# kevlar-dev/kevlar

Measured on AMD Instinct MI355X. Metric: reads/sec through count+novel (3 samples, k=31), higher is better.
Workload: dtype u64 hash / u8 counters

## Files before the change

### kevlar_amd/csrc/kv_binned.hip

```cpp
#include <algorithm>
#include <cmath>
#include <map>
#include <type_traits>

#include "kv_binned.h"
#include "kv_device.h"
#include "kv_kmer2bit_device.h"

namespace {

#define BIN_RING_MIN 64
#define BIN_RING_MAX 4096
#define BIN_B_THREADS 512
#define BIN_B_ITEMS 8
#define BIN_B_BUDGET 16384
#define BIN_C_THREADS 1024
#define BIN_MAX_SEG 512

template <typename ItemT>
struct Rings {
    ItemT *ring;
    uint32_t *cnt, *base;
    uint32_t R;
    uint32_t skew;
// ... 263 lines not shown
        __syncthreads();
        const uint64_t i0 = next_chunk * chunk;
        if (i0 >= n) break;
        uint64_t idx = i0 + threadIdx.x;
        uint64_t h_next = idx < n ? list[idx * stride] : 0, c_next = (W && idx < n) ? list[idx * stride + 1] : 1;
        for (int round = 0; round < BIN_LIST_ROUNDS; ++round) {
            const uint64_t h = h_next, count = c_next;
            const bool live = idx < n;
            idx += THREADS;
            if (round + 1 < BIN_LIST_ROUNDS && idx < n) {
                h_next = list[idx * stride];
                if (W) c_next = list[idx * stride + 1];
            }
            if (!live) continue;
            n_added += count;
            uint32_t left = W ? (uint32_t)min(count, (uint64_t)255) : 1u;
            while (left) {
                const uint32_t wgt = W ? min(left, BIN_W_MAX) : 1u;
                left -= wgt;
                uint32_t sidx[BIN_MAX_T], item[BIN_MAX_T], pos[BIN_MAX_T];
                uint64_t bins[BIN_MAX_T];
#pragma unroll
                for (int t = 0; t < BIN_MAX_T; ++t) {
                    if (t >= g.T) break;
                    const uint64_t bin = fastmod(h, sk->size[t], sk->magic[t]);
                    const uint32_t slice = (uint32_t)(bin >> g.sbits);
                    const uint32_t c = g.F == 1 ? slice : __umulhi(slice, g.recipF);
                    bins[t] = bin;
                    item[t] = ((slice - c * (uint32_t)g.F) << g.sbits) | ((uint32_t)bin & ((1u << g.sbits) - 1u)) | (W ? (wgt - 1u) << BIN_W_SHIFT : 0u);
                    sidx[t] = (uint32_t)t * (uint32_t)g.C + c;
                }
#pragma unroll
                for (int t = 0; t < BIN_MAX_T; ++t)
                    if (t < g.T) pos[t] = atomicAdd(&cur[sidx[t]], 1u);
#pragma unroll
                for (int t = 0; t < BIN_MAX_T; ++t) {
                    if (t >= g.T) break;
                    if (pos[t] < g.cap1) g.gbuf1[((uint64_t)sidx[t] * g.nwgA + blockIdx.x) * g.cap1 + pos[t]] = item[t];
                    else spill_item(g, t, bins[t], wgt);
                }
            }
        }
    }
    __syncthreads();
    for (uint32_t s = threadIdx.x; s < ns; s += THREADS)
        g.gcnt1[(uint64_t)s * g.nwgA + blockIdx.x] = (uint32_t)min((uint64_t)cur[s], g.cap1);
    if (W) {
        n_added = wave_sum_u64(n_added);
        if ((threadIdx.x & 63) == 0 && n_added) atomicAdd(&g.ctr[2], (unsigned long long)n_added);
    }
}

template <bool W>
__global__ __launch_bounds__(BIN_B_THREADS) void k_bin_split(BinGeom g)
{
    typedef typename std::conditional<W, uint32_t, uint16_t>::type Out;
    extern __shared__ __attribute__((aligned(16))) unsigned char smem[];
    const uint32_t s = blockIdx.y;
    const uint32_t t = s / (uint32_t)g.C, c = s % (uint32_t)g.C;
    const uint32_t F = (uint32_t)g.F;
    Rings<Out> rs;
    rs.R = g.ringB;
    rs.skew = 8;
    rs.ring = (Out *)smem;
    rs.cnt = (uint32_t *)(smem + (((size_t)F * rs.R * sizeof(Out) + 15) & ~(size_t)15));
    rs.base = rs.cnt + F;
    for (uint32_t i = threadIdx.x; i < F; i += BIN_B_THREADS) { rs.cnt[i] = 0; rs.base[i] = 0; }
    __syncthreads();
    uint32_t written = 0;
    uint64_t seg_base = 0;
    {
        const uint32_t nwaves = BIN_B_THREADS >> 6, per_wave = (F + nwaves - 1) / nwaves;
        const uint32_t mine = (threadIdx.x >> 6) * per_wave + (threadIdx.x & 63);
        if ((threadIdx.x & 63) < per_wave && mine < F) seg_base = (((uint64_t)s * F + mine) * g.nwgB + blockIdx.x) * g.cap2;
    }
    Out *gbuf2 = (Out *)g.gbuf2;
    constexpr uint32_t SB = BIN_SLICE_BITS, OFFMASK = (1u << SB) - 1u;
    auto slice_of = [](uint32_t item) { return W ? (item >> SB) & ((1u << (BIN_W_SHIFT - SB)) - 1u) : item >> SB; };
    auto fine_of = [](uint32_t item) { return W ? (Out)((item & OFFMASK) | (((item >> BIN_W_SHIFT) + 1u) << 16)) : (Out)(item & OFFMASK); };
    auto spill_coarse = [&](uint32_t item) {
        spill_item(g, (int)t, (((uint64_t)c * F + slice_of(item)) << SB) | (item & OFFMASK), W ? (item >> BIN_W_SHIFT) + 1u : 1u);
    };
    auto store = [&](uint64_t idx, Out off) { gbuf2[idx] = off; };
    auto overflow = [&](uint32_t fi, Out off) {
        spill_item(g, (int)t, (((uint64_t)c * F + fi) << SB) | ((uint32_t)off & OFFMASK), W ? (uint32_t)off >> 16 : 1u);
    };
    constexpr int ITEMS = W ? 4 : BIN_B_ITEMS;
    const uint64_t step = (uint64_t)BIN_B_THREADS * ITEMS;
    for (uint32_t seg = blockIdx.x; seg < g.nwgA; seg += g.nwgB) {
        uint64_t end = g.gcnt1[(uint64_t)s * g.nwgA + seg];
        if (end > g.cap1) end = g.cap1;
        const uint32_t *src = g.gbuf1 + ((uint64_t)s * g.nwgA + seg) * g.cap1;
        uint4 va = make_uint4(0, 0, 0, 0), vb = va;
        auto fetch = [&](uint64_t r0, uint4 &a, uint4 &b) {
            const uint64_t i0 = r0 + (uint64_t)threadIdx.x * ITEMS;
            if (i0 + ITEMS <= end) { a = *(const uint4 *)(src + i0); if (ITEMS == 8) b = *(const uint4 *)(src + i0 + 4); }
        };
        fetch(0, va, vb);
        for (uint64_t r0 = 0; r0 < end; r0 += step) {
            const uint64_t i0 = r0 + (uint64_t)threadIdx.x * ITEMS;
            uint32_t items[ITEMS];
            int have = 0;
            if (i0 + ITEMS <= end) {
                items[0] = va.x; items[1] = va.y; items[2] = va.z; items[3] = va.w;
                if (ITEMS == 8) { items[ITEMS - 4] = vb.x; items[ITEMS - 3] = vb.y; items[ITEMS - 2] = vb.z; items[ITEMS - 1] = vb.w; }
                have = ITEMS;
            } else {
                for (uint64_t i = i0; i < end; ++i) items[have++] = src[i];
            }
            if (r0 + step < end) fetch(r0 + step, va, vb);
            if (have == ITEMS) {
                uint32_t pos[ITEMS], rbase[ITEMS];
#pragma unroll
                for (int j = 0; j < ITEMS; ++j) pos[j] = atomicAdd(&rs.cnt[slice_of(items[j])], 1u);
#pragma unroll
                for (int j = 0; j < ITEMS; ++j) rbase[j] = rs.base[slice_of(items[j])];
                uint32_t full = 0;
#pragma unroll
                for (int j = 0; j < ITEMS; ++j) {
                    const uint32_t fi = slice_of(items[j]);
                    if (pos[j] - rbase[j] < rs.R) rs.ring[fi * rs.R + ((pos[j] + rs.skew * fi) & (rs.R - 1))] = fine_of(items[j]);
                    else full |= 1u << j;
                }
                if (full) {
#pragma unroll
                    for (int j = 0; j < ITEMS; ++j)
                        if (full & (1u << j)) spill_coarse(items[j]);
                }
            } else {
                for (int j = 0; j < have; ++j)
                    if (!ring_append(rs, slice_of(items[j]), fine_of(items[j]))) spill_coarse(items[j]);
            }
            __syncthreads();
            rings_flush_lanes(rs, F, written, seg_base, (uint32_t)g.cap2, gbuf2, overflow);
            __syncthreads();
        }
    }
    rings_flush(rs, F, true, written, seg_base, (uint32_t)g.cap2, store, overflow, 64u / (uint32_t)sizeof(Out));
    rings_store_counts(F, written, (uint32_t)g.cap2, g.gcnt2 + (uint64_t)s * F * g.nwgB, g.nwgB, blockIdx.x);
}

__device__ __forceinline__ bool lds_inc(uint32_t *lds, uint32_t off, int storage)
{
    if (storage == ST_BIT) {
        const uint32_t bit = 1u << (off & 31);
        return (atomicOr(&lds[off >> 5], bit) & bit) == 0;
    }
    uint32_t *w;
    uint32_t shift, maxv;
    if (storage == ST_BYTE) {
        w = &lds[off >> 2]; shift = (off & 3) * 8u; maxv = 255u;
    } else {
        const uint32_t byte = off >> 1;
        w = &lds[byte >> 2]; shift = (byte & 3) * 8u + ((off & 1) ? 0u : 4u); maxv = 15u;
    }
    uint32_t old = *w;
    for (;;) {
        const uint32_t cur = (old >> shift) & maxv;
        if (cur == maxv) return false;
        const uint32_t prev = atomicCAS(w, old, old + (1u << shift));
        if (prev == old) return cur == 0;
        old = prev;
    }
}

template <int STORAGE>
__device__ __forceinline__ uint32_t lds_inc8(uint32_t *lds, const uint32_t (&w)[4], uint32_t n)
{
    uint32_t fresh = 0;
    if (STORAGE == ST_BIT) {
#pragma unroll
        for (int e = 0; e < 8; ++e) {
            const uint32_t off = (e & 1) ? (w[e >> 1] >> 16) : (w[e >> 1] & 0xffffu);
            if ((uint32_t)e < n) {
                const uint32_t bit = 1u << (off & 31);
                fresh += (atomicOr(&lds[off >> 5], bit) & bit) == 0 ? 1u : 0u;
            }
        }
        return fresh;
    }
    constexpr uint32_t maxv = STORAGE == ST_BYTE ? 255u : 15u;
    uint32_t widx[8], inc[8], old[8], prev[8];
    uint32_t retry = 0;
#pragma unroll
    for (int e = 0; e < 8; ++e) {
        const uint32_t off = (e & 1) ? (w[e >> 1] >> 16) : (w[e >> 1] & 0xffffu);
        uint32_t shift;
        if (STORAGE == ST_BYTE) { widx[e] = off >> 2; shift = (off & 3u) << 3; }
        else { widx[e] = off >> 3; shift = (((off >> 1) & 3u) << 3) + ((off & 1u) ? 0u : 4u); }
        inc[e] = 1u << shift;
    }
#pragma unroll
// ... 39 lines not shown
        for (int e = 0; e < 4; ++e) {
            const uint32_t off = w[e] & 0xffffu;
            if ((uint32_t)e < n) {
                const uint32_t bit = 1u << (off & 31);
                fresh += (atomicOr(&lds[off >> 5], bit) & bit) == 0 ? 1u : 0u;
            }
        }
        return fresh;
    }
    constexpr uint32_t maxv = STORAGE == ST_BYTE ? 255u : 15u;
    uint32_t widx[4], shift[4], add[4], old[4], prev[4];
    bool live[4];
    uint32_t retry = 0;
#pragma unroll
    for (int e = 0; e < 4; ++e) {
        const uint32_t off = w[e] & 0xffffu;
        add[e] = w[e] >> 16;
        if (STORAGE == ST_BYTE) { widx[e] = off >> 2; shift[e] = (off & 3u) << 3; }
        else { widx[e] = off >> 3; shift[e] = (((off >> 1) & 3u) << 3) + ((off & 1u) ? 0u : 4u); }
    }
#pragma unroll
    for (int e = 0; e < 4; ++e) old[e] = lds[widx[e]];
#pragma unroll
    for (int e = 0; e < 4; ++e) {
        const uint32_t field = (old[e] >> shift[e]) & maxv;
        const uint32_t nf = min(maxv, field + add[e]);
        live[e] = (uint32_t)e < n && nf != field;
        prev[e] = atomicCAS(&lds[widx[e]], old[e], old[e] + (live[e] ? (nf - field) << shift[e] : 0u));
    }
#pragma unroll
    for (int e = 0; e < 4; ++e) {
        const bool won = prev[e] == old[e];
        fresh += (live[e] && won && ((old[e] >> shift[e]) & maxv) == 0) ? 1u : 0u;
        retry |= (live[e] && !won) ? (1u << e) : 0u;
    }
    if (retry) {
#pragma unroll
        for (int e = 0; e < 4; ++e) {
            if (!(retry & (1u << e))) continue;
            uint32_t cur_word = prev[e];
            for (;;) {
                const uint32_t field = (cur_word >> shift[e]) & maxv;
                if (field == maxv) break;
                const uint32_t nf = min(maxv, field + add[e]);
                const uint32_t seen = atomicCAS(&lds[widx[e]], cur_word, cur_word + ((nf - field) << shift[e]));
                if (seen == cur_word) { fresh += field == 0 ? 1u : 0u; break; }
                cur_word = seen;
            }
        }
    }
    return fresh;
}

template <int STORAGE, bool W>
__global__ __launch_bounds__(BIN_C_THREADS) void k_bin_apply(const SketchDev *__restrict__ sk, BinGeom g)
{
    typedef typename std::conditional<W, uint32_t, uint16_t>::type Item;
    constexpr uint32_t VEC = 16u / sizeof(Item);
    constexpr uint32_t SB = BIN_SLICE_BITS, SLICE = 1u << SB;
    constexpr uint32_t THREADS = BIN_C_THREADS;
    constexpr int MAXV = W ? 4 : 3;
    __shared__ __attribute__((aligned(16))) uint32_t lds[SLICE / 4];
    const int t = blockIdx.y;
    const uint32_t slice = blockIdx.x;
    if (slice >= g.nslices[t]) return;
    const uint32_t c = slice / (uint32_t)g.F, fidx = slice % (uint32_t)g.F;
    const uint64_t stream = ((uint64_t)t * g.C + c) * g.F + fidx;
    constexpr int storage = STORAGE;
    const uint64_t bin0 = (uint64_t)slice << SB;
    const uint64_t left = g.tsize[t] - bin0, nb = left < SLICE ? left : SLICE;
    const uint64_t byte0 = storage == ST_BYTE ? bin0 : (storage == ST_NIBBLE ? bin0 >> 1 : bin0 >> 3);
    const uint64_t nbytes = storage == ST_BYTE ? nb : (storage == ST_NIBBLE ? (nb + 1) / 2 : (nb + 7) / 8);
    const uint32_t nvec = (uint32_t)((nbytes + 15) / 16);
    uint4 *tab = (uint4 *)(g.ttab[t] + byte0);
    uint4 *l4 = (uint4 *)lds;
    __shared__ uint32_t seg_cnt[BIN_MAX_SEG], vpre[BIN_MAX_SEG];
    __shared__ uint16_t segof[MAXV * THREADS];
    __shared__ uint32_t wsum[THREADS / 64];
    __shared__ uint32_t total_vec_sh, flag_sh, fresh_sh;
    const Item *items = (const Item *)g.gbuf2 + stream * g.nwgB * g.cap2;
    const uint32_t *counts = g.gcnt2 + stream * g.nwgB;
    {
        uint32_t myc = 0;
        if (threadIdx.x < g.nwgB) myc = counts[threadIdx.x];
        unsigned long long flag = 0;
        if (threadIdx.x == THREADS - 1) flag = g.ctr[1];
        if (!g.zero_tables)
            for (uint32_t j = threadIdx.x; j < nvec; j += THREADS) l4[j] = tab[j];
        if (threadIdx.x < g.nwgB) seg_cnt[threadIdx.x] = myc;
        const uint32_t myv = (myc + VEC - 1) / VEC;
        const int lane = threadIdx.x & 63, wave = threadIdx.x >> 6;
        uint32_t incl = myv;
#pragma unroll
        for (int d = 1; d < 64; d <<= 1) {
            const uint32_t up = __shfl_up(incl, d);
            if (lane >= d) incl += up;
        }
        if (lane == 63) wsum[wave] = incl;
        if (threadIdx.x == THREADS - 1) { flag_sh = flag != 0 ? 1u : 0u; fresh_sh = 0; }
        __syncthreads();
        uint32_t before = 0;
        for (int w = 0; w < wave; ++w) before += wsum[w];
        if (threadIdx.x < g.nwgB) vpre[threadIdx.x] = before + incl - myv;
        if (threadIdx.x == THREADS - 1) total_vec_sh = before + incl;
        __syncthreads();
        for (uint32_t sgi = (uint32_t)wave; sgi < g.nwgB; sgi += THREADS / 64) {
            const uint32_t first = vpre[sgi], nv = (seg_cnt[sgi] + VEC - 1) / VEC;
            for (uint32_t i = (uint32_t)lane; i < nv && first + i < (uint32_t)MAXV * THREADS; i += 64) segof[first + i] = (uint16_t)sgi;
        }
        __syncthreads();
    }
    if (flag_sh) return;
    const uint32_t total_vec = total_vec_sh;
    if (total_vec == 0) {
        if (g.zero_tables)
            for (uint32_t j = threadIdx.x; j < nvec; j += THREADS) tab[j] = make_uint4(0, 0, 0, 0);
        return;
    }
    struct Vec { uint4 q; uint32_t n; };
    auto fetch = [&](uint32_t v) {
        Vec r;
        r.q = make_uint4(0, 0, 0, 0); r.n = 0;
        if (v >= total_vec) return r;
        uint32_t lo = 0, hi = g.nwgB;
        if (v < (uint32_t)MAXV * THREADS) {
            lo = segof[v];
        } else {
            while (hi - lo > 1) {
                const uint32_t mid = (lo + hi) >> 1;
                if (vpre[mid] <= v) lo = mid; else hi = mid;
            }
        }
        const uint32_t j0 = (v - vpre[lo]) * VEC;
        r.n = min(VEC, seg_cnt[lo] - j0);
        r.q = *(const uint4 *)(items + (uint64_t)lo * g.cap2 + j0);
        return r;
    };
    Vec first[MAXV];
#pragma unroll
    for (int i = 0; i < MAXV; ++i) first[i] = fetch(threadIdx.x + (uint32_t)i * THREADS);
    if (g.zero_tables)
        for (uint32_t j = threadIdx.x; j < nvec; j += THREADS) l4[j] = make_uint4(0, 0, 0, 0);
    __syncthreads();
    uint32_t fresh = 0;
#pragma unroll
    for (int i = 0; i < MAXV; ++i) {
        const uint32_t w[4] = {first[i].q.x, first[i].q.y, first[i].q.z, first[i].q.w};
        if (first[i].n) fresh += W ? lds_addw4<STORAGE>(lds, w, first[i].n) : lds_inc8<STORAGE>(lds, w, first[i].n);
    }
    if (total_vec > (uint32_t)MAXV * THREADS) {
        const uint32_t v_start = (uint32_t)MAXV * THREADS + threadIdx.x;
        Vec v0 = fetch(v_start), v1 = fetch(v_start + THREADS);
        for (uint32_t v = v_start; v < total_vec; v += THREADS) {
            const Vec v2 = fetch(v + 2 * THREADS);
            const uint32_t w[4] = {v0.q.x, v0.q.y, v0.q.z, v0.q.w};
            fresh += W ? lds_addw4<STORAGE>(lds, w, v0.n) : lds_inc8<STORAGE>(lds, w, v0.n);
            v0 = v1; v1 = v2;
        }
    }
    if (t == 0) {
        const uint32_t tot = (uint32_t)wave_sum_u64(fresh);
        if ((threadIdx.x & 63) == 0 && tot) atomicAdd(&fresh_sh, tot);
    }
    __syncthreads();
    for (uint32_t j = threadIdx.x; j < nvec; j += THREADS) tab[j] = l4[j];
    if (t == 0 && threadIdx.x == 0 && fresh_sh) atomicAdd(&g.ctr[3], (unsigned long long)fresh_sh);
}

__device__ __forceinline__ bool table_add_bin(const SketchDev *s, int t, uint64_t bin, uint32_t weight)
{
    uint8_t *tab = s->tab[t];
    if (s->storage == ST_BIT) {
        const uint32_t bit = 1u << (bin & 31);
        return (atomicOr((uint32_t *)tab + (bin >> 5), bit) & bit) == 0;
    }
    uint32_t *w;
    uint32_t shift, maxv;
    if (s->storage == ST_BYTE) {
        w = (uint32_t *)(tab + (bin & ~3ull)); shift = (uint32_t)(bin & 3) * 8u; maxv = 255u;
    } else {
        const uint64_t byte = bin >> 1;
        w = (uint32_t *)(tab + (byte & ~3ull)); shift = (uint32_t)(byte & 3) * 8u + ((bin & 1) ? 0u : 4u); maxv = 15u;
    }
    uint32_t old = __hip_atomic_load(w, __ATOMIC_RELAXED, __HIP_MEMORY_SCOPE_AGENT);
    for (;;) {
        const uint32_t cur = (old >> shift) & maxv;
        if (cur == maxv) return false;
        const uint32_t nf = min(maxv, cur + weight);
        const uint32_t prev = atomicCAS(w, old, old + ((nf - cur) << shift));
        if (prev == old) return cur == 0;
        old = prev;
    }
}

__global__ void k_bin_spill(const SketchDev *__restrict__ sk, BinGeom g)
{
    if (g.ctr[1] != 0) return;
    unsigned long long n = g.ctr[0];
    if (n > g.spill_cap) n = g.spill_cap;
    uint64_t fresh = 0;
    for (uint64_t i = blockIdx.x * (uint64_t)blockDim.x + threadIdx.x; i < n; i += (uint64_t)gridDim.x * blockDim.x) {
        const unsigned long long e = g.spill[i];
        const int t = (int)((e >> 32) & 0xffu);
        const bool was_zero = table_add_bin(sk, t, e & 0xffffffffull, (uint32_t)((e >> 40) & 0xffu) + 1u);
        fresh += (was_zero && t == 0) ? 1 : 0;
    }
    fresh = wave_sum_u64(fresh);
    if ((threadIdx.x & 63) == 0 && fresh) atomicAdd(&g.ctr[3], (unsigned long long)fresh);
}

std::map<hipStream_t, KvArena> g_scratch;
std::mutex g_scratch_mu;

KvArena &scratch_for(hipStream_t st)
{
    std::lock_guard<std::mutex> lk(g_scratch_mu);
    return g_scratch[kv_stream_key(st)];
}
}
void kv_bin_scratch_release()
{
    std::lock_guard<std::mutex> lk(g_scratch_mu);
    for (auto &kv : g_scratch) kv.second.release();
}
namespace {

template <typename K>
void ensure_dynamic_lds(K kernel, size_t bytes) { kv_ensure_dynamic_lds((const void *)kernel, bytes); }

}

int kv_device_cus()
{
    static int cus = 0;
    if (cus == 0) {
        int dev = 0, n = 256;
        kv_thread_device();
        (void)hipGetDevice(&dev);
        (void)hipDeviceGetAttribute(&n, hipDeviceAttributeMultiprocessorCount, dev);
        cus = n;
    }
    return cus;
}

double kv_estimate_distinct(uint64_t occupied, uint64_t size)
{
    if (occupied >= size) return (double)size * std::log((double)size);
    return -(double)size * std::log1p(-(double)occupied / (double)size);
}

bool kv_bin_two_bit(const kv_sketch *s, const kv_reads *reads)
{
    const char *e = kv_knob("KV_BIN_2BIT");
    if (e && atoi(e) == 0) return false;
    return reads && reads->uni_len != 0 && reads->uni_per_tile != 0 && s->h.hashfam == HF_MURMUR && s->h.ksize >= SKM_MIN_K && s->h.ksize <= SKM_MAX_K &&
           reads->uni_len >= (uint32_t)s->h.ksize && reads->n_tiles > 0;
}

bool kv_binned_eligible(const kv_sketch *s, const kv_reads *reads, uint64_t n_kmers, int nbands)
{
    const char *force = kv_knob("KV_COUNT_PATH");
    if (force && strcmp(force, "atomic") == 0) return false;
    if (s->h.ntables > BIN_MAX_T) return false;
    uint64_t pmin = UINT64_MAX, pmax = 0;
    for (int t = 0; t < s->h.ntables; ++t) { pmin = std::min(pmin, s->h.size[t]); pmax = std::max(pmax, s->h.size[t]); }
    if (pmax > (uint64_t)BIN_C * BIN_MAX_F * 65536ull) return false;
    if (force && (strcmp(force, "binned") == 0 || strcmp(force, "skm") == 0)) return reads ? reads->n_tiles > 0 : n_kmers > 0;
    const uint64_t expected = nbands > 0 ? n_kmers / (uint64_t)nbands : n_kmers;
    const uint64_t density = !reads || kv_bin_two_bit(s, reads) ? 32 : 8;
    return pmin >= (1ull << 20) && expected >= (1ull << 22) && expected * density >= pmax;
}

int kv_bin_plan(kv_sketch *s, uint64_t n_items_max, int nbands, bool use_mask, uint64_t work_units, uint32_t lds_front,
                uint32_t nwgA_fixed, bool weighted, BinPlan *plan)
{
    hipStream_t st = kv_stream();
    KvArena &scratch = scratch_for(st);
    BinGeom &g = plan->g;
    memset(&g, 0, sizeof(g));
    plan->weighted = weighted;
    g.zero_tables = s->lazy_zero ? 1 : 0;
// ... 24 lines not shown
    plan->threadsA = threadsA;
    if (nwgA_fixed) g.nwgA = nwgA_fixed;
    else g.nwgA = (uint32_t)std::min<uint64_t>(std::max<uint64_t>(work_units, 1), (cmax <= 32 ? 3u : 1u) * (uint32_t)cus);
    {
        const uint64_t avg = (std::max<uint64_t>(work_units, 1) + g.nwgA - 1) / g.nwgA;
        g.quotaA = (uint32_t)std::min<uint64_t>(avg + avg / 2 + 1, 0xffffffffull);
    }
    const double slice_bins = (double)(1u << g.sbits);
    const double per_bucket = expected * std::min(1.0, (double)g.F * slice_bins / (double)pmin);
    const double per_slice = expected * std::min(1.0, slice_bins / (double)pmin);
    g.nwgB = (uint32_t)std::max(1.0, std::min((double)std::min<uint32_t>(g.nwgA, 512), std::ceil(per_bucket / 524288.0)));
    g.nwgB = std::max<uint32_t>(g.nwgB, std::min<uint32_t>(std::min<uint32_t>(g.nwgA, 512), (g.nwgA + 31u) / 32u));
    const double m1 = per_bucket / g.nwgA, m2 = per_slice / g.nwgB;
    g.cap1 = kv_round_up((uint64_t)(m1 * 1.5 + 8.0 * std::sqrt(m1)) + 2048, 64);
    g.cap2 = kv_round_up((uint64_t)(m2 * 1.05 + 8.0 * std::sqrt(m2)) + 64, 64);
    g.spill_cap = std::max<uint64_t>(1u << 22, (uint64_t)(expected * g.T / 8));
    const size_t fine_bytes = weighted ? 4 : 2;
    const size_t b_buf1 = kv_round_up(ns * g.nwgA * g.cap1 * 4, 256), b_buf2 = kv_round_up(ns * g.F * g.nwgB * g.cap2 * fine_bytes, 256);
    const size_t b_cnt1 = kv_round_up(ns * g.nwgA * 4, 256), b_cnt2 = kv_round_up(ns * g.F * g.nwgB * 4, 256);
    const size_t b_spill = kv_round_up(g.spill_cap * 8, 256), b_ctr = 256;
    if (scratch.need(b_buf1 + b_buf2 + b_cnt1 + b_cnt2 + b_spill + b_ctr) != hipSuccess) {
        (void)hipGetLastError();
        kv_set_error("no device memory for the partitioned count's staging buffers (%.1f GB)", (double)(b_buf1 + b_buf2 + b_cnt1 + b_cnt2 + b_spill + b_ctr) / 1e9);
        return KV_ERR_CAPACITY;
    }
    unsigned char *base = (unsigned char *)scratch.p;
    g.gbuf1 = (uint32_t *)base; base += b_buf1;
    g.gbuf2 = (uint16_t *)base; base += b_buf2;
    g.gcnt1 = (uint32_t *)base; base += b_cnt1;
    g.gcnt2 = (uint32_t *)base; base += b_cnt2;
    g.spill = (unsigned long long *)base; base += b_spill;
    g.ctr = (unsigned long long *)base;
    {
        bool ok = g.T == 4 && ns * g.nwgA * g.cap1 < (1ull << 32);
        for (int t = 0; t < g.T && t < BIN_MAX_T; ++t) {
            g.tmagic[t] = kv_fastmod_magic(s->h.size[t]);
            ok = ok && kv_fastmod_fp(s->h.size[t]) && s->h.size[t] < (1ull << 31);
        }
        g.fast4 = ok ? 1 : 0;
    }
    KV_HIP(hipMemsetAsync(g.ctr, 0, b_ctr, st));
    return KV_OK;
}

int kv_bin_finish(kv_sketch *s, BinPlan &plan, bool added_from_ctr, uint64_t n_added_fixed, uint64_t *n_added)
{
    hipStream_t st = kv_stream();
    BinGeom &g = plan.g;
    const uint64_t ns = (uint64_t)g.T * g.C;
    {
        KvProfScope prof(plan.weighted ? "k_bin_split_w" : "k_bin_split");
        const size_t isz = plan.weighted ? 4 : 2;
        const size_t lds = (((size_t)g.F * g.ringB * isz + 15) & ~(size_t)15) + (size_t)g.F * 2 * 4;
        if (plan.weighted) {
            ensure_dynamic_lds((k_bin_split<true>), lds);
            hipLaunchKernelGGL((k_bin_split<true>), dim3(g.nwgB, (unsigned)ns), dim3(BIN_B_THREADS), lds, st, g);
        } else {
            ensure_dynamic_lds((k_bin_split<false>), lds);
            hipLaunchKernelGGL((k_bin_split<false>), dim3(g.nwgB, (unsigned)ns), dim3(BIN_B_THREADS), lds, st, g);
        }
    }
    {
        KvProfScope prof(plan.weighted ? "k_bin_apply_w" : "k_bin_apply");
        const dim3 gridC(plan.maxsl, (unsigned)g.T);
        const SketchDev *d = (const SketchDev *)s->d_desc;
#define KV_LAUNCH_APPLY(ST_, W_) \
        hipLaunchKernelGGL((k_bin_apply<ST_, W_>), gridC, dim3(BIN_C_THREADS), 0, st, d, g)
#define KV_LAUNCH_APPLY_ST(W_)                                               \
        do {                                                                  \
            if (s->h.storage == ST_BYTE) KV_LAUNCH_APPLY(ST_BYTE, W_);        \
            else if (s->h.storage == ST_NIBBLE) KV_LAUNCH_APPLY(ST_NIBBLE, W_); \
            else KV_LAUNCH_APPLY(ST_BIT, W_);                                 \
        } while (0)
        if (plan.weighted) KV_LAUNCH_APPLY_ST(true);
        else KV_LAUNCH_APPLY_ST(false);
#undef KV_LAUNCH_APPLY_ST
#undef KV_LAUNCH_APPLY
    }
    {
        KvProfScope prof("k_bin_spill");
        hipLaunchKernelGGL(k_bin_spill, dim3(256), dim3(256), 0, st, (const SketchDev *)s->d_desc, g);
    }
    KV_HIP(hipGetLastError());
    unsigned long long ctr[4] = {0, 0, 0, 0};
    KV_HIP(hipMemcpyAsync(ctr, g.ctr, sizeof(ctr), hipMemcpyDeviceToHost, st));
    KV_HIP(hipStreamSynchronize(st));
    if (ctr[1] != 0) {
        kv_set_error("partitioned count: spill list overflow (%llu items)", ctr[0]);
        return KV_ERR_CAPACITY;
    }
    *n_added = added_from_ctr ? ctr[2] : n_added_fixed;
    s->lazy_zero = false;
    if (s->occ_dirty) {
        int rc = kv_sketch_refresh_occupancy(s);
        if (rc != KV_OK) return rc;
        s->n_unique = (uint64_t)(kv_estimate_distinct(s->n_occupied, s->h.size[0]) + 0.5);
    } else {
        const double before = kv_estimate_distinct(s->n_occupied, s->h.size[0]);
        s->n_occupied += ctr[3];
        const double after = kv_estimate_distinct(s->n_occupied, s->h.size[0]);
        s->n_unique += (uint64_t)(after - before + 0.5);
    }
    return KV_OK;
}

int kv_consume_binned(kv_sketch *s, const kv_reads *reads, const uint64_t *d_list, uint32_t list_stride,
                      const ConsumeFilter &filter, const kv_sketch *mask, uint64_t n_kmers, int nbands, uint64_t *n_added,
                      bool weighted_list)
{
    hipStream_t st = kv_stream();
    BinPlan plan;
    const bool two_bit = reads && kv_bin_two_bit(s, reads);
    const uint32_t n_units2 = two_bit ? (reads->n_tiles + BIN2_TILES - 1u) / BIN2_TILES : 0u;
    {
        uint32_t maxsl = 1;
        for (int t = 0; t < s->h.ntables; ++t) maxsl = std::max(maxsl, (uint32_t)((s->h.size[t] + 65535) >> 16));
        const uint32_t threadsA = maxsl <= 32u * BIN_MAX_F ? 512u : 1024u;
        const uint64_t work_units = two_bit ? n_units2 : reads ? reads->n_tiles
                                          : (n_kmers + (uint64_t)threadsA * BIN_LIST_ROUNDS - 1) / ((uint64_t)threadsA * BIN_LIST_ROUNDS);
        const int rc = kv_bin_plan(s, n_kmers, nbands, filter.use_mask != 0, work_units, reads && !two_bit ? reads->tile_lds_bytes : 0u, 0u, weighted_list, &plan);
// ... 48 lines not shown
```

### kevlar_amd/csrc/kv_host.hip

```cpp
#include <algorithm>
#include <functional>
#include <atomic>
#include <cstdarg>
#include <map>

#include "kv_internal.h"

static thread_local char g_err[512] = "";
thread_local int kv_last_hip_code = 0;

void kv_set_error(const char *fmt, ...)
{
    va_list ap;
    va_start(ap, fmt);
    vsnprintf(g_err, sizeof(g_err), fmt, ap);
    va_end(ap);
}

uint64_t kv_next_uid()
{
    static std::atomic<uint64_t> next{1};
    return next.fetch_add(1);
}

// ... 1066 lines not shown
    if (r->d_woff) (void)hipFree(r->d_woff);
    if (r->d_len) (void)hipFree(r->d_len);
    if (r->d_flags) (void)hipFree(r->d_flags);
    if (r->d_tile) (void)hipFree(r->d_tile);
    delete r;
    return KV_OK;
}

extern "C" int kv_reads_count(const kv_reads *r, uint64_t *n_reads, uint64_t *n_bases)
{
    KV_REQUIRE(r, KV_ERR_ARG, "kv_reads_count: null handle");
    if (n_reads) *n_reads = r->n_reads;
    if (n_bases) *n_bases = r->n_bases;
    return KV_OK;
}

extern "C" int kv_reads_num_kmers(const kv_reads *r, int ksize, uint64_t *n_kmers)
{
    KV_REQUIRE(r && n_kmers && ksize >= 1, KV_ERR_ARG, "kv_reads_num_kmers: bad argument");
    if (r->nk_cached_k != ksize) {
        uint64_t n = 0;
        for (uint32_t len : r->h_len)
            if (len >= (uint32_t)ksize) n += len - (uint32_t)ksize + 1;
        kv_reads *w = const_cast<kv_reads *>(r);
        w->nk_cached = n;
        w->nk_cached_k = ksize;
    }
    *n_kmers = r->nk_cached;
    return KV_OK;
}

namespace {
#define S_ KV_KNOB_SETTING
#define T_ KV_KNOB_TUNING
const KvKnobDef g_knobs[] = {
    {"KV_TABLE_CACHE_GB", S_, "table buffers of destroyed sketches kept for the next sketch of the same size, in GB (default 32; 0: none)"},
    {"KV_AUGFASTX_THREADS", S_, "host threads of the augmented FASTX reader / writer (default: by input size, up to the cores)"},
    {"KV_FORMAT_THREADS", S_, "host threads formatting annotated reads (default: min(16, cores))"},
    {"KV_STAGE_THREADS", S_, "host threads reading a file into the pinned staging buffers (1..16)"},
    {"KEVLAR_PACK_CACHE", S_, "packed-read cache files beside the inputs: unset / 0 never, 1 use and create"},
    {"KV_INGEST", S_, "host: parse every file on the host, never on the device"},
    {"KV_GUNZIP", S_, "host: ordinary gzip streams through zlib on the host instead of the device inflater (BGZF and plain FASTQ stay on the device)"},
    {"KV_GUNZIP_CRC", S_, "0: skip the CRC-32 check of inflated members"},
    {"KV_PARALLEL_SAMPLES", S_, "1 / 0: count the samples of `kevlar novel` side by side on their own streams / one after the other"},
    {"KV_INGEST_VERBOSE", S_, "wall time of every ingest step on stderr"},
    {"KV_GUNZIP_VERBOSE", S_, "statistics of the gzip inflater on stderr"},
    {"KV_SKM_VERBOSE", S_, "what the super-k-mer front end decided (geometry, lists kept or dropped, fallbacks) on stderr"},
    {"KV_MEX_VERBOSE", S_, "why a rank declined a step of the exchange layout, on stderr"},
    {"KV_COUNT_PATH", T_, "atomic | binned | skm: pin the count path"},
    {"KV_NOVEL_PATH", T_, "tiles | skm: pin the scan path"},
    {"KV_ROUTE_PATH", T_, "plain: the exchange routes one item per k-mer (no combining)"},
    {"KV_SET_SCAN", T_, "skm: a shard's set scan keeps the bucketed kernel"},
    {"KV_BIN_2BIT", T_, "0: stage A never hashes from the 2-bit form"},
    {"KV_SKM_S2", T_, "plain | sorted: pin the fine split"},
    {"KV_SKM_ANY_K", T_, "use the kernels with k at run time, not the k = 31 / 51 instances"},
    {"KV_SKM_BUCKET_KMERS", T_, "k-mer occurrences aimed at per bucket (tests: many buckets on small inputs)"},
    {"KV_SKM_CAP_PCT", T_, "segment capacity in per cent of the estimate (tests: push records through the loose list)"},
    {"KV_SKM_LOOSE_CAP", T_, "entries of the loose list"},
    {"KV_SKM_FORCE_LOOSE", T_, "one key in 64 is counted as if its table were full: its occurrences travel through the loose list"},
    {"KV_SKM_DL", T_, "0: no distinct list from a case sample's count; 1: from the first batch on"},
    {"KV_SKM_NO_REUSE", T_, "the scan re-buckets the batch instead of reusing the count's buckets"},
    {"KV_NOVEL_2BIT", T_, "0: the per-k-mer scan keeps the tile kernel"},
    {"KV_NOVEL_BITS", T_, "0: no bit map as the first probe of the scan"},
    {"KV_NOVEL_BITS_MIN", T_, "items from which the pairs scan builds its bit map"},
    {"KV_NOVEL_PAIRS", T_, "0: the set scan answers from hashes alone"},
    {"KV_NOVEL_REREAD", T_, "`kevlar novel` reads a case file again for the scan instead of keeping its batch"},
    {"KV_HOST_SORT", T_, "partition sorts its keys on the host"},
    {"KV_STAGE", T_, "0: uploads straight from the file mapping, no pinned staging"},
    {"KV_INGEST_TEXT_MB", T_, "text per ingest batch in MB (tests: small batches)"},
    {"KV_GUNZIP_TEXT_MIN_MB", T_, "gzip files from this size on are inflated on the device"},
    {"KV_GUNZIP_CHUNK_KB", T_, "1..64: compressed bytes per probe stretch"},
    {"KV_MEX_PASSES", T_, "exchange: combine passes per bucket, at least (1-16)"},
    {"KV_MEX_DL_POOL", T_, "exchange: 1 = the owner's distinct list as a pool of chunks at once (it is the last resort of an owner short of memory)"},
    {"KV_MEX_PAIRS", T_, "9: (hash, count) pairs travel in the 9-byte block form"},
    {"KV_MEX_TEST_DECLINE", T_, "point:rank -- that rank fails at that point of the exchange (tests of the agreed fallbacks)"},
    {"KV_ALLBANDS_TEST_FAIL", T_, "rank:band -- `novel --all-bands`: that rank fails before counting that band (0-based; test of the agreed stop)"},
    {"KV_ROUTE_OVF_CAP", T_, "entries of the route's overflow list (tests: force the capacity error)"},
};
#undef S_
#undef T_
}

const KvKnobDef *kv_knob_table(size_t *n)
{
    if (n) *n = sizeof(g_knobs) / sizeof(g_knobs[0]);
    return g_knobs;
}

static bool knob_honoured(KvKnobClass cls)
{
    if (cls == KV_KNOB_SETTING) return true;
    const char *t = getenv("KV_TUNING");
    return t && atoi(t) == 1;
}

const char *kv_knob(const char *name)
{
    for (const KvKnobDef &d : g_knobs)
        if (!strcmp(d.name, name)) return knob_honoured(d.cls) ? getenv(name) : nullptr;
    fprintf(stderr, "[kvsketch] kv_knob(\"%s\"): not in the registry of kv_host.hip\n", name);
    return nullptr;
}

extern "C" int kv_knob_get(const char *name, char *value_out, uint64_t cap)
{
    KV_REQUIRE(name, KV_ERR_ARG, "kv_knob_get: null name");
// ... 28 lines not shown
```

Measured before the change: 1.013 billion.

## Make binned split and apply kernels persistent with cross-unit prefetch

The split and apply kernels of the binned count path now launch a grid sized from occupancy times the number of CUs, and each workgroup loops over several work units instead of one unit per block. The split kernel prefetches the first vector of the next segment while it finishes the current one. The apply kernel loads the next unit's segment counts early and reuses its LDS table across units. The aim is to cut block launch and tail overhead and to hide load latency, at the cost of more complex per-unit state resets and less parallelism when there are few units.

After: 989.5 million. 2.3% lower.

```diff
diff --git a/kevlar_amd/csrc/kv_binned.hip b/kevlar_amd/csrc/kv_binned.hip
--- a/kevlar_amd/csrc/kv_binned.hip
+++ b/kevlar_amd/csrc/kv_binned.hip
@@ -339,12 +339,10 @@
 }
 
 template <bool W>
-__global__ __launch_bounds__(BIN_B_THREADS) void k_bin_split(BinGeom g)
+__global__ __launch_bounds__(BIN_B_THREADS) void k_bin_split(BinGeom g, uint32_t n_units)
 {
     typedef typename std::conditional<W, uint32_t, uint16_t>::type Out;
     extern __shared__ __attribute__((aligned(16))) unsigned char smem[];
-    const uint32_t s = blockIdx.y;
-    const uint32_t t = s / (uint32_t)g.C, c = s % (uint32_t)g.C;
     const uint32_t F = (uint32_t)g.F;
     Rings<Out> rs;
     rs.R = g.ringB;
@@ -352,15 +350,34 @@
     rs.ring = (Out *)smem;
     rs.cnt = (uint32_t *)(smem + (((size_t)F * rs.R * sizeof(Out) + 15) & ~(size_t)15));
     rs.base = rs.cnt + F;
+    struct Cursor { uint32_t unit, seg; };
+    auto advance = [&](Cursor x) {
+        x.seg += g.nwgB;
+        if (x.seg >= g.nwgA) { x.unit += gridDim.x; x.seg = x.unit % g.nwgB; }
+        return x;
+    };
+    auto live = [&](const Cursor &x) { return x.unit < n_units; };
+    auto slot_of = [&](const Cursor &x) { return (uint64_t)(x.unit / g.nwgB) * g.nwgA + x.seg; };
+    auto count_of = [&](const Cursor &x) { return (uint32_t)min((uint64_t)g.gcnt1[slot_of(x)], g.cap1); };
+    Cursor c0 = {blockIdx.x, blockIdx.x % g.nwgB};
+    if (!live(c0)) return;
+    Cursor c1 = advance(c0);
+    uint32_t end = count_of(c0), end1 = live(c1) ? count_of(c1) : 0u;
     for (uint32_t i = threadIdx.x; i < F; i += BIN_B_THREADS) { rs.cnt[i] = 0; rs.base[i] = 0; }
     __syncthreads();
+    const uint32_t nwaves = BIN_B_THREADS >> 6, per_wave = (F + nwaves - 1) / nwaves;
+    const uint32_t mine = (threadIdx.x >> 6) * per_wave + (threadIdx.x & 63);
+    const bool owner = (threadIdx.x & 63) < per_wave && mine < F;
+    uint32_t s = 0, w = 0, t = 0, c = 0;
     uint32_t written = 0;
     uint64_t seg_base = 0;
-    {
-        const uint32_t nwaves = BIN_B_THREADS >> 6, per_wave = (F + nwaves - 1) / nwaves;
-        const uint32_t mine = (threadIdx.x >> 6) * per_wave + (threadIdx.x & 63);
-        if ((threadIdx.x & 63) < per_wave && mine < F) seg_base = (((uint64_t)s * F + mine) * g.nwgB + blockIdx.x) * g.cap2;
-    }
+    auto begin_unit = [&](uint32_t unit) {
+        s = unit / g.nwgB; w = unit % g.nwgB;
+        t = s / (uint32_t)g.C; c = s % (uint32_t)g.C;
+        written = 0;
+        seg_base = owner ? (((uint64_t)s * F + mine) * g.nwgB + w) * g.cap2 : 0;
+    };
+    begin_unit(c0.unit);
     Out *gbuf2 = (Out *)g.gbuf2;
     constexpr uint32_t SB = BIN_SLICE_BITS, OFFMASK = (1u << SB) - 1u;
     auto slice_of = [](uint32_t item) { return W ? (item >> SB) & ((1u << (BIN_W_SHIFT - SB)) - 1u) : item >> SB; };
@@ -373,19 +390,20 @@
         spill_item(g, (int)t, (((uint64_t)c * F + fi) << SB) | ((uint32_t)off & OFFMASK), W ? (uint32_t)off >> 16 : 1u);
     };
     constexpr int ITEMS = W ? 4 : BIN_B_ITEMS;
-    const uint64_t step = (uint64_t)BIN_B_THREADS * ITEMS;
-    for (uint32_t seg = blockIdx.x; seg < g.nwgA; seg += g.nwgB) {
-        uint64_t end = g.gcnt1[(uint64_t)s * g.nwgA + seg];
-        if (end > g.cap1) end = g.cap1;
-        const uint32_t *src = g.gbuf1 + ((uint64_t)s * g.nwgA + seg) * g.cap1;
-        uint4 va = make_uint4(0, 0, 0, 0), vb = va;
-        auto fetch = [&](uint64_t r0, uint4 &a, uint4 &b) {
-            const uint64_t i0 = r0 + (uint64_t)threadIdx.x * ITEMS;
-            if (i0 + ITEMS <= end) { a = *(const uint4 *)(src + i0); if (ITEMS == 8) b = *(const uint4 *)(src + i0 + 4); }
-        };
-        fetch(0, va, vb);
-        for (uint64_t r0 = 0; r0 < end; r0 += step) {
-            const uint64_t i0 = r0 + (uint64_t)threadIdx.x * ITEMS;
+    const uint32_t step = (uint32_t)BIN_B_THREADS * ITEMS;
+    uint4 va = make_uint4(0, 0, 0, 0), vb = va;
+    auto fetch = [&](const uint32_t *from, uint32_t upto, uint32_t r0, uint4 &a, uint4 &b) {
+        const uint64_t i0 = (uint64_t)r0 + threadIdx.x * ITEMS;
+        if (i0 + ITEMS <= upto) { a = *(const uint4 *)(from + i0); if (ITEMS == 8) b = *(const uint4 *)(from + i0 + 4); }
+    };
+    bool ahead = false;
+    for (;;) {
+        const uint32_t *src = g.gbuf1 + slot_of(c0) * g.cap1;
+        const uint32_t *src1 = live(c1) ? g.gbuf1 + slot_of(c1) * g.cap1 : src;
+        if (!ahead) fetch(src, end, 0, va, vb);
+        ahead = false;
+        for (uint32_t r0 = 0; r0 < end; r0 += step) {
+            const uint64_t i0 = (uint64_t)r0 + threadIdx.x * ITEMS;
             uint32_t items[ITEMS];
             int have = 0;
             if (i0 + ITEMS <= end) {
@@ -395,7 +413,8 @@
             } else {
                 for (uint64_t i = i0; i < end; ++i) items[have++] = src[i];
             }
-            if (r0 + step < end) fetch(r0 + step, va, vb);
+            if (r0 + step < end) fetch(src, end, r0 + step, va, vb);
+            else if (end1) { fetch(src1, end1, 0, va, vb); ahead = true; }
             if (have == ITEMS) {
                 uint32_t pos[ITEMS], rbase[ITEMS];
 #pragma unroll
@@ -422,9 +441,21 @@
             rings_flush_lanes(rs, F, written, seg_base, (uint32_t)g.cap2, gbuf2, overflow);
             __syncthreads();
         }
-    }
-    rings_flush(rs, F, true, written, seg_base, (uint32_t)g.cap2, store, overflow, 64u / (uint32_t)sizeof(Out));
-    rings_store_counts(F, written, (uint32_t)g.cap2, g.gcnt2 + (uint64_t)s * F * g.nwgB, g.nwgB, blockIdx.x);
+        const bool more = live(c1), unit_ends = !more || c1.unit != c0.unit;
+        if (unit_ends) {
+            rings_flush(rs, F, true, written, seg_base, (uint32_t)g.cap2, store, overflow, 64u / (uint32_t)sizeof(Out));
+            rings_store_counts(F, written, (uint32_t)g.cap2, g.gcnt2 + (uint64_t)s * F * g.nwgB, g.nwgB, w);
+            if (owner) { rs.cnt[mine] = 0; rs.base[mine] = 0; }
+        }
+        if (!more) break;
+        if (unit_ends) {
+            __syncthreads();
+            begin_unit(c1.unit);
+        }
+        c0 = c1; end = end1;
+        c1 = advance(c1);
+        end1 = live(c1) ? count_of(c1) : 0u;
+    }
 }
 
 __device__ __forceinline__ bool lds_inc(uint32_t *lds, uint32_t off, int storage)
@@ -570,44 +601,60 @@
     return fresh;
 }
 
+template <int STORAGE, bool W, bool FRESH>
+__device__ __forceinline__ uint32_t bin_apply_vec(uint32_t *lds, const uint4 &q, uint32_t n)
+{
+    const uint32_t w[4] = {q.x, q.y, q.z, q.w};
+    const uint32_t fresh = W ? lds_addw4<STORAGE>(lds, w, n) : lds_inc8<STORAGE>(lds, w, n);
+    return FRESH ? fresh : 0u;
+}
+
 template <int STORAGE, bool W>
-__global__ __launch_bounds__(BIN_C_THREADS) void k_bin_apply(const SketchDev *__restrict__ sk, BinGeom g)
+__global__ __launch_bounds__(BIN_C_THREADS, 8) void k_bin_apply(const SketchDev *__restrict__ sk, BinGeom g, uint32_t n_units)
 {
     typedef typename std::conditional<W, uint32_t, uint16_t>::type Item;
     constexpr uint32_t VEC = 16u / sizeof(Item);
     constexpr uint32_t SB = BIN_SLICE_BITS, SLICE = 1u << SB;
     constexpr uint32_t THREADS = BIN_C_THREADS;
     constexpr int MAXV = W ? 4 : 3;
+    constexpr int storage = STORAGE;
     __shared__ __attribute__((aligned(16))) uint32_t lds[SLICE / 4];
-    const int t = blockIdx.y;
-    const uint32_t slice = blockIdx.x;
-    if (slice >= g.nslices[t]) return;
-    const uint32_t c = slice / (uint32_t)g.F, fidx = slice % (uint32_t)g.F;
-    const uint64_t stream = ((uint64_t)t * g.C + c) * g.F + fidx;
-    constexpr int storage = STORAGE;
-    const uint64_t bin0 = (uint64_t)slice << SB;
-    const uint64_t left = g.tsize[t] - bin0, nb = left < SLICE ? left : SLICE;
-    const uint64_t byte0 = storage == ST_BYTE ? bin0 : (storage == ST_NIBBLE ? bin0 >> 1 : bin0 >> 3);
-    const uint64_t nbytes = storage == ST_BYTE ? nb : (storage == ST_NIBBLE ? (nb + 1) / 2 : (nb + 7) / 8);
-    const uint32_t nvec = (uint32_t)((nbytes + 15) / 16);
-    uint4 *tab = (uint4 *)(g.ttab[t] + byte0);
-    uint4 *l4 = (uint4 *)lds;
     __shared__ uint32_t seg_cnt[BIN_MAX_SEG], vpre[BIN_MAX_SEG];
     __shared__ uint16_t segof[MAXV * THREADS];
     __shared__ uint32_t wsum[THREADS / 64];
-    __shared__ uint32_t total_vec_sh, flag_sh, fresh_sh;
-    const Item *items = (const Item *)g.gbuf2 + stream * g.nwgB * g.cap2;
-    const uint32_t *counts = g.gcnt2 + stream * g.nwgB;
-    {
-        uint32_t myc = 0;
-        if (threadIdx.x < g.nwgB) myc = counts[threadIdx.x];
-        unsigned long long flag = 0;
-        if (threadIdx.x == THREADS - 1) flag = g.ctr[1];
-        if (!g.zero_tables)
-            for (uint32_t j = threadIdx.x; j < nvec; j += THREADS) l4[j] = tab[j];
-        if (threadIdx.x < g.nwgB) seg_cnt[threadIdx.x] = myc;
+    __shared__ uint32_t total_vec_sh, fresh_sh;
+    uint4 *l4 = (uint4 *)lds;
+    uint32_t tid = threadIdx.x;
+    const uint32_t stride = gridDim.x;
+    uint32_t u = blockIdx.x;
+    if (u >= n_units) return;
+    if (g.ctr[1] != 0) return;
+
+    struct Unit { int t; uint32_t nvec; uint4 *tab; const Item *items; const uint32_t *counts; };
+    auto unit_of = [&](uint32_t unit) {
+        Unit x;
+        uint32_t slice = unit;
+        int t = 0;
+#pragma unroll
+        for (int i = 0; i + 1 < BIN_MAX_T; ++i)
+            if (t == i && slice >= g.nslices[i]) { slice -= g.nslices[i]; t = i + 1; }
+        const uint32_t c = slice / (uint32_t)g.F, fidx = slice % (uint32_t)g.F;
+        const uint64_t stream = ((uint64_t)t * g.C + c) * g.F + fidx;
+        const uint64_t bin0 = (uint64_t)slice << SB;
+        const uint64_t left = g.tsize[t] - bin0, nb = left < SLICE ? left : SLICE;
+        const uint64_t byte0 = storage == ST_BYTE ? bin0 : (storage == ST_NIBBLE ? bin0 >> 1 : bin0 >> 3);
+        const uint64_t nbytes = storage == ST_BYTE ? nb : (storage == ST_NIBBLE ? (nb + 1) / 2 : (nb + 7) / 8);
+        x.t = t;
+        x.nvec = (uint32_t)((nbytes + 15) / 16);
+        x.tab = (uint4 *)(g.ttab[t] + byte0);
+        x.items = (const Item *)g.gbuf2 + stream * g.nwgB * g.cap2;
+        x.counts = g.gcnt2 + stream * g.nwgB;
+        return x;
+    };
+    auto build = [&](uint32_t myc) {
+        const int lane = tid & 63, wave = tid >> 6;
+        if (tid < g.nwgB) seg_cnt[tid] = myc;
         const uint32_t myv = (myc + VEC - 1) / VEC;
-        const int lane = threadIdx.x & 63, wave = threadIdx.x >> 6;
         uint32_t incl = myv;
 #pragma unroll
         for (int d = 1; d < 64; d <<= 1) {
@@ -615,28 +662,22 @@
             if (lane >= d) incl += up;
         }
         if (lane == 63) wsum[wave] = incl;
-        if (threadIdx.x == THREADS - 1) { flag_sh = flag != 0 ? 1u : 0u; fresh_sh = 0; }
         __syncthreads();
         uint32_t before = 0;
         for (int w = 0; w < wave; ++w) before += wsum[w];
-        if (threadIdx.x < g.nwgB) vpre[threadIdx.x] = before + incl - myv;
-        if (threadIdx.x == THREADS - 1) total_vec_sh = before + incl;
+        if (tid < g.nwgB) vpre[tid] = before + incl - myv;
+        if (tid == THREADS - 1) total_vec_sh = before + incl;
         __syncthreads();
         for (uint32_t sgi = (uint32_t)wave; sgi < g.nwgB; sgi += THREADS / 64) {
             const uint32_t first = vpre[sgi], nv = (seg_cnt[sgi] + VEC - 1) / VEC;
             for (uint32_t i = (uint32_t)lane; i < nv && first + i < (uint32_t)MAXV * THREADS; i += 64) segof[first + i] = (uint16_t)sgi;
         }
         __syncthreads();
-    }
-    if (flag_sh) return;
-    const uint32_t total_vec = total_vec_sh;
-    if (total_vec == 0) {
-        if (g.zero_tables)
-            for (uint32_t j = threadIdx.x; j < nvec; j += THREADS) tab[j] = make_uint4(0, 0, 0, 0);
-        return;
-    }
+        return (uint32_t)__builtin_amdgcn_readfirstlane((int)total_vec_sh);
+    };
     struct Vec { uint4 q; uint32_t n; };
-    auto fetch = [&](uint32_t v) {
+    struct VecSet { uint4 q[MAXV]; uint32_t n; };
+    auto fetch = [&](const Item *items, uint32_t total_vec, uint32_t v) {
         Vec r;
         r.q = make_uint4(0, 0, 0, 0); r.n = 0;
         if (v >= total_vec) return r;
@@ -654,35 +695,73 @@
         r.q = *(const uint4 *)(items + (uint64_t)lo * g.cap2 + j0);
         return r;
     };
-    Vec first[MAXV];
-#pragma unroll
-    for (int i = 0; i < MAXV; ++i) first[i] = fetch(threadIdx.x + (uint32_t)i * THREADS);
+    auto counts_of = [&](const Unit &x) { return tid < g.nwgB ? x.counts[tid] : 0u; };
+
+    auto fetch_set = [&](const Item *items, uint32_t total_vec, VecSet &x) {
+        x.n = 0;
+#pragma unroll
+        for (int i = 0; i < MAXV; ++i) {
+            const Vec r = fetch(items, total_vec, tid + (uint32_t)i * THREADS);
+            x.q[i] = r.q;
+            x.n |= r.n << (4 * i);
+        }
+    };
+    Unit cu = unit_of(u);
+    uint32_t myc = counts_of(cu);
     if (g.zero_tables)
-        for (uint32_t j = threadIdx.x; j < nvec; j += THREADS) l4[j] = make_uint4(0, 0, 0, 0);
+        for (uint32_t j = tid; j < SLICE / 16; j += THREADS) l4[j] = make_uint4(0, 0, 0, 0);
+    if (tid == THREADS - 1) fresh_sh = 0;
+    uint32_t fresh = 0;
+    for (;;) {
+        asm volatile("" : "+v"(tid));
+        const uint32_t tv = build(myc);
+        VecSet cur;
+        fetch_set(cu.items, tv, cur);
+        const bool have_next = u + stride < n_units;
+        Unit nx = cu;
+        myc = 0;
+        if (have_next) { nx = unit_of(u + stride); myc = counts_of(nx); }
+        if (!g.zero_tables && tv) {
+            for (uint32_t j = tid; j < cu.nvec; j += THREADS) l4[j] = cu.tab[j];
+            __syncthreads();
+        }
+        if (tv) {
+            if (cu.t == 0) {
+#pragma unroll
+                for (int i = 0; i < MAXV; ++i)
+                    if ((cur.n >> (4 * i)) & 15u) fresh += bin_apply_vec<STORAGE, W, true>(lds, cur.q[i], (cur.n >> (4 * i)) & 15u);
+            } else {
+#pragma unroll
+                for (int i = 0; i < MAXV; ++i)
+                    if ((cur.n >> (4 * i)) & 15u) bin_apply_vec<STORAGE, W, false>(lds, cur.q[i], (cur.n >> (4 * i)) & 15u);
+            }
+            if (tv > (uint32_t)MAXV * THREADS) {
+                const uint32_t v_start = (uint32_t)MAXV * THREADS + tid;
+                Vec v0 = fetch(cu.items, tv, v_start), v1 = fetch(cu.items, tv, v_start + THREADS);
+                for (uint32_t v = v_start; v < tv; v += THREADS) {
+                    const Vec v2 = fetch(cu.items, tv, v + 2 * THREADS);
+                    if (cu.t == 0) fresh += bin_apply_vec<STORAGE, W, true>(lds, v0.q, v0.n);
+                    else bin_apply_vec<STORAGE, W, false>(lds, v0.q, v0.n);
+                    v0 = v1; v1 = v2;
+                }
+            }
+            __syncthreads();
+            if (g.zero_tables) {
+                for (uint32_t j = tid; j < cu.nvec; j += THREADS) { cu.tab[j] = l4[j]; l4[j] = make_uint4(0, 0, 0, 0); }
+            } else {
+                for (uint32_t j = tid; j < cu.nvec; j += THREADS) cu.tab[j] = l4[j];
+            }
+        } else if (g.zero_tables) {
+            for (uint32_t j = tid; j < cu.nvec; j += THREADS) cu.tab[j] = make_uint4(0, 0, 0, 0);
+        }
+        if (!have_next) break;
+        u += stride;
+        cu = nx;
+    }
+    const uint32_t tot = (uint32_t)wave_sum_u64(fresh);
+    if ((tid & 63) == 0 && tot) atomicAdd(&fresh_sh, tot);
     __syncthreads();
-    uint32_t fresh = 0;
-#pragma unroll
-    for (int i = 0; i < MAXV; ++i) {
-        const uint32_t w[4] = {first[i].q.x, first[i].q.y, first[i].q.z, first[i].q.w};
-        if (first[i].n) fresh += W ? lds_addw4<STORAGE>(lds, w, first[i].n) : lds_inc8<STORAGE>(lds, w, first[i].n);
-    }
-    if (total_vec > (uint32_t)MAXV * THREADS) {
-        const uint32_t v_start = (uint32_t)MAXV * THREADS + threadIdx.x;
-        Vec v0 = fetch(v_start), v1 = fetch(v_start + THREADS);
-        for (uint32_t v = v_start; v < total_vec; v += THREADS) {
-            const Vec v2 = fetch(v + 2 * THREADS);
-            const uint32_t w[4] = {v0.q.x, v0.q.y, v0.q.z, v0.q.w};
-            fresh += W ? lds_addw4<STORAGE>(lds, w, v0.n) : lds_inc8<STORAGE>(lds, w, v0.n);
-            v0 = v1; v1 = v2;
-        }
-    }
-    if (t == 0) {
-        const uint32_t tot = (uint32_t)wave_sum_u64(fresh);
-        if ((threadIdx.x & 63) == 0 && tot) atomicAdd(&fresh_sh, tot);
-    }
-    __syncthreads();
-    for (uint32_t j = threadIdx.x; j < nvec; j += THREADS) tab[j] = l4[j];
-    if (t == 0 && threadIdx.x == 0 && fresh_sh) atomicAdd(&g.ctr[3], (unsigned long long)fresh_sh);
+    if (tid == 0 && fresh_sh) atomicAdd(&g.ctr[3], (unsigned long long)fresh_sh);
 }
 
 __device__ __forceinline__ bool table_add_bin(const SketchDev *s, int t, uint64_t bin, uint32_t weight)
@@ -745,6 +824,30 @@
 
 template <typename K>
 void ensure_dynamic_lds(K kernel, size_t bytes) { kv_ensure_dynamic_lds((const void *)kernel, bytes); }
+
+template <typename K>
+uint32_t persistent_grid(K kernel, int threads, size_t dyn_lds, uint32_t units)
+{
+    static std::mutex mu;
+    static std::map<size_t, int> per_cu;
+    int n = 0;
+    {
+        std::lock_guard<std::mutex> lk(mu);
+        auto it = per_cu.find(dyn_lds);
+        if (it == per_cu.end()) {
+            kv_thread_device();
+            if (hipOccupancyMaxActiveBlocksPerMultiprocessor(&n, (const void *)kernel, threads, dyn_lds) != hipSuccess || n < 1) {
+                (void)hipGetLastError();
+                n = 1;
+            }
+            it = per_cu.emplace(dyn_lds, n).first;
+        }
+        n = it->second;
+    }
+    uint64_t grid = std::min<uint64_t>(std::max<uint32_t>(units, 1u), (uint64_t)n * (uint64_t)kv_device_cus());
+    if (const char *e = kv_knob("KV_BIN_WGS")) grid = std::min<uint64_t>(grid, (uint64_t)std::max(1, atoi(e)));
+    return (uint32_t)grid;
+}
 
 }
 
@@ -875,20 +978,22 @@
         KvProfScope prof(plan.weighted ? "k_bin_split_w" : "k_bin_split");
         const size_t isz = plan.weighted ? 4 : 2;
         const size_t lds = (((size_t)g.F * g.ringB * isz + 15) & ~(size_t)15) + (size_t)g.F * 2 * 4;
+        const uint32_t units = (uint32_t)ns * g.nwgB;
         if (plan.weighted) {
             ensure_dynamic_lds((k_bin_split<true>), lds);
-            hipLaunchKernelGGL((k_bin_split<true>), dim3(g.nwgB, (unsigned)ns), dim3(BIN_B_THREADS), lds, st, g);
+            hipLaunchKernelGGL((k_bin_split<true>), dim3(persistent_grid(k_bin_split<true>, BIN_B_THREADS, lds, units)), dim3(BIN_B_THREADS), lds, st, g, units);
         } else {
             ensure_dynamic_lds((k_bin_split<false>), lds);
-            hipLaunchKernelGGL((k_bin_split<false>), dim3(g.nwgB, (unsigned)ns), dim3(BIN_B_THREADS), lds, st, g);
+            hipLaunchKernelGGL((k_bin_split<false>), dim3(persistent_grid(k_bin_split<false>, BIN_B_THREADS, lds, units)), dim3(BIN_B_THREADS), lds, st, g, units);
         }
     }
     {
         KvProfScope prof(plan.weighted ? "k_bin_apply_w" : "k_bin_apply");
-        const dim3 gridC(plan.maxsl, (unsigned)g.T);
+        uint32_t units = 0;
+        for (int t = 0; t < g.T; ++t) units += g.nslices[t];
         const SketchDev *d = (const SketchDev *)s->d_desc;
 #define KV_LAUNCH_APPLY(ST_, W_) \
-        hipLaunchKernelGGL((k_bin_apply<ST_, W_>), gridC, dim3(BIN_C_THREADS), 0, st, d, g)
+        hipLaunchKernelGGL((k_bin_apply<ST_, W_>), dim3(persistent_grid(k_bin_apply<ST_, W_>, BIN_C_THREADS, 0, units)), dim3(BIN_C_THREADS), 0, st, d, g, units)
 #define KV_LAUNCH_APPLY_ST(W_)                                               \
         do {                                                                  \
             if (s->h.storage == ST_BYTE) KV_LAUNCH_APPLY(ST_BYTE, W_);        \
diff --git a/kevlar_amd/csrc/kv_host.hip b/kevlar_amd/csrc/kv_host.hip
--- a/kevlar_amd/csrc/kv_host.hip
+++ b/kevlar_amd/csrc/kv_host.hip
@@ -1142,6 +1142,7 @@
     {"KV_ROUTE_PATH", T_, "plain: the exchange routes one item per k-mer (no combining)"},
     {"KV_SET_SCAN", T_, "skm: a shard's set scan keeps the bucketed kernel"},
     {"KV_BIN_2BIT", T_, "0: stage A never hashes from the 2-bit form"},
+    {"KV_BIN_WGS", T_, "most workgroups of the persistent split and apply kernels (tests: several units per workgroup on small tables)"},
     {"KV_SKM_S2", T_, "plain | sorted: pin the fine split"},
     {"KV_SKM_ANY_K", T_, "use the kernels with k at run time, not the k = 31 / 51 instances"},
     {"KV_SKM_BUCKET_KMERS", T_, "k-mer occurrences aimed at per bucket (tests: many buckets on small inputs)"},
```
